# angelini/raft-simulation

Hardware: AMD Instinct MI355X
Metric: simulated node-ticks/sec (5-node Raft) (higher is better)
Workload: dtype u32; 1 GPU; C2: 65,536 5-node clusters/GPU, 10k ticks/step, no faults, no client (steady window); clusters=65536, clusters_per_gpu=65536, nodes=5, parallelism=cluster-sharded x1

## Files before the change

### raft-simulation_amd/csrc/steady_kernel.hip

```cpp
#include <hip/hip_ext.h>

#include "fixed_point_affine.hpp"
#include "tick_wave.hpp"

namespace rs {

constexpr int LANE_WG = 256;

template <int N>
__device__ __forceinline__ uint32_t pick(const uint32_t (&vals)[N], uint32_t k) {
  uint32_t v = 0;
#pragma unroll
  for (int i = 0; i < N; ++i) v |= vals[i] & (0u - (uint32_t)(k == (uint32_t)i));
  return v;
}
__device__ __forceinline__ uint32_t msel(bool a, uint32_t x, uint32_t y) {
  const uint32_t m = 0u - (uint32_t)a;
  return (x & m) | (y & ~m);
}

constexpr int IMG_SLOTS = 32;
constexpr uint32_t IMG_LINE = 64 * 8 * 16;
constexpr uint32_t IMG_HALF = 2 * IMG_LINE;
constexpr uint32_t IMG_WAVE = 2 * IMG_HALF;
// ... 14 lines not shown
}

template <int n>
__host__ __device__ constexpr uint64_t trace_pow() {
  uint64_t x = 1;
  for (int i = 0; i < n; ++i) x *= TRACE_M2;
  return x;
}
template <int n>
__host__ __device__ constexpr uint64_t trace_geo() {
  uint64_t s = 0, x = 1;
  for (int i = 0; i < n; ++i) {
    s += x;
    x *= TRACE_M2;
  }
  return s;
}

static_assert(fpa::M == TRACE_M && fpa::M2 == TRACE_M2 && fpa::ROLE_LEADER == RAFT_LEADER &&
                  fpa::ROLE_FOLLWER == RAFT_FOLLWER &&
                  fpa::EV_APPEND_ENTRIES == RAFT_MSG_APPEND_ENTRIES &&
                  fpa::EV_APPEND_RESPONSE == RAFT_MSG_APPEND_RESPONSE,
              "the affine step's hash is the trace hash");

struct alignas(16) SetWords {
  uint64_t la, lx, ly, lz, fa, fx, fy, fz;
  uint32_t ls, fs, K, K1;
  __device__ __forceinline__ fpa::Half lead() const { return fpa::Half{la, lx, ly, lz, ls}; }
  __device__ __forceinline__ fpa::Half fol() const { return fpa::Half{fa, fx, fy, fz, fs}; }
};
struct BandSets {
  SetWords k[2];
};
__device__ __forceinline__ uint32_t vreg(uint32_t s) {
  uint32_t v;
  asm volatile("v_mov_b32 %0, %1" : "=v"(v) : "s"(s));
  return v;
}
__device__ __forceinline__ uint64_t vreg(uint64_t s) {
  return (uint64_t)vreg((uint32_t)(s >> 32)) << 32 | vreg((uint32_t)s);
}
__device__ __forceinline__ SetWords vreg(const fpa::Set& c, uint32_t K1) {
  return SetWords{vreg(c.lead.a), vreg(c.lead.x), vreg(c.lead.y), vreg(c.lead.z),
                  vreg(c.fol.a),  vreg(c.fol.x),  vreg(c.fol.y),  vreg(c.fol.z),
                  vreg(c.lead.s), vreg(c.fol.s),  vreg(c.K),      vreg(K1)};
}
template <int F>
__device__ __forceinline__ void band_sets(uint32_t nt, uint32_t d, uint32_t hb, BandSets* out) {
  const uint32_t P = fpa::period(F, d, hb), last = 2 * d + F - 1;
  const uint32_t K1 = nt > last ? (nt - last - 1) / P + 1 : 0;
  const fpa::Set lo = fpa::build<F>(d, hb, K1 ? K1 - 1 : 0), hi = fpa::step<F>(lo, d, hb);
  out->k[0] = vreg(lo, K1);
  out->k[1] = vreg(hi, K1);
}

template <int N>
struct FixedPoint {
  static constexpr int F = N - 1;
  uint32_t L, Lid, Lterm, Lcommit;
  uint64_t Ltr, ftr[F];
  uint32_t Ldl, fdl[F], fpend;
  uint32_t qmask, qA[F], qT[F], qa[F], qb[F];
  uint32_t rmask, resA, rT[F], rA[F], rB[F], rH[F];
  uint32_t nhb, nae, nar;

  __device__ __forceinline__ uint32_t fk(int j) const { return (uint32_t)j + ((uint32_t)j >= L ? 1u : 0u); }

  __device__ __forceinline__ void append_entries(uint32_t ta, uint32_t d, uint32_t el_base) {
#pragma unroll
    for (int j = 0; j < F; ++j) {
      ftr[j] = trace_event(ftr[j], ta, RAFT_MSG_APPEND_ENTRIES, Lid, Lterm, RAFT_FOLLWER, Lterm, 0);
      fdl[j] = ta + el_base;
      rT[j] = Lterm; rA[j] = Lcommit; rB[j] = 0; rH[j] = 1;
      qA[j] = INF;
    }
    fpend = (1u << F) - 1;
    qmask = 0;
    rmask = (1u << F) - 1;
    resA = ta + d;
    nae += F;
  }
  __device__ __forceinline__ void responses(uint32_t th, uint32_t tend, uint32_t d, uint32_t hb) {
#pragma unroll
    for (int j = 0; j < F; ++j) {
      const uint32_t tau = th + 2 * d + j;
      if (((rmask >> j) & 1) && tau < tend) {
        Ltr = trace_event(Ltr, tau, RAFT_MSG_APPEND_RESPONSE, fk(j) + 1, Lterm, RAFT_LEADER,
                          Lterm, 0);
        rmask &= ~(1u << j);
        Ldl = tau + hb;
        ++nar;
      }
    }
    if (!rmask) resA = INF;
  }
  __device__ __forceinline__ void rounds(uint32_t th, uint32_t tend, uint32_t d, uint32_t hb,
                                         uint32_t el_base, const BandSets& bs) {
    const uint32_t P = 2 * d + F - 1 + hb, last = 2 * d + F - 1;
    const uint32_t K = tend > th + last ? (tend - th - last - 1) / P + 1 : 0;
    const uint32_t tk = th + K * P;
    if (K) {
      const uint32_t K1 = bs.k[0].K1;
      const bool top = K == K1;
      if (!__builtin_amdgcn_ballot_w64(!top && K + 1 != K1)) {
        const SetWords sw = bs.k[top];
        const fpa::Half cl = sw.lead(), cf = sw.fol();
        Ltr = fpa::apply_leader<F>(cl, Ltr, th, Lterm, L);
        const uint64_t add = fpa::follower_addend<F>(cf, th, Lterm, L);
#pragma unroll
        for (int j = 0; j < F; ++j) ftr[j] = ftr[j] * cf.a + add;
      } else {
        uint64_t a = trace_term(th, 7, 0, 0, RAFT_LEADER, Lterm, 0);
#pragma unroll
        for (int j = 0; j < F; ++j)
          a = a * TRACE_M2 + trace_term(th + 2 * d + j, RAFT_MSG_APPEND_RESPONSE, fk(j) + 1, Lterm,
                                        RAFT_LEADER, Lterm, 0);
        const uint64_t da = (uint64_t)P * (TRACE_M * trace_geo<F + 1>());
        const uint64_t df = (uint64_t)P * TRACE_M;
        uint64_t cf = trace_term(th + d, RAFT_MSG_APPEND_ENTRIES, Lid, Lterm, RAFT_FOLLWER, Lterm, 0);
        for (uint32_t r = 0; r < K; ++r) {
          Ltr = Ltr * trace_pow<F + 1>() + a;
          a += da;
#pragma unroll
          for (int j = 0; j < F; ++j) ftr[j] = ftr[j] * TRACE_M2 + cf;
          cf += df;
        }
      }
#pragma unroll
      for (int j = 0; j < F; ++j) fdl[j] = tk - P + d + el_base;
      fpend = (1u << F) - 1;
      Ldl = tk;
      nhb += K;
      nae += F * K;
      nar += F * K;
    }
    if (tk < tend) {
      Ltr = trace_event(Ltr, tk, 7, 0, 0, RAFT_LEADER, Lterm, 0);
      ++nhb;
      Ldl = tk + hb;
#pragma unroll
      for (int j = 0; j < F; ++j) {
        qA[j] = tk + d; qT[j] = Lterm; qa[j] = Lcommit; qb[j] = 0;
      }
      qmask = (1u << F) - 1;
      if (tk + d < tend) {
        append_entries(tk + d, d, el_base);
        responses(tk, tend, d, hb);
      }
    }
  }
};

template <int N>
__global__ void __launch_bounds__(LANE_WG) steady_lane_kernel(DevSim S, uint32_t t0, uint32_t nt) {
  static_assert(N >= 2 && N <= 5, "follower masks and the response queue fit four followers");
  constexpr int F = N - 1;
  constexpr uint32_t HB = hot_block_words(N);
  constexpr int NWORDS = (int)(HOT_CW + hf_abase(N) * N);
  constexpr int NW4 = (NWORDS + 3) / 4;
  constexpr int IMGC = (int)(HB / 4) < IMG_SLOTS ? (int)(HB / 4) : IMG_SLOTS;
  static_assert(NW4 <= IMGC && IMGC % 8 == 0, "the image holds the words read, in whole lines");
  __shared__ uint32_t bl_c[LANE_WG], bl_t[LANE_WG];
  __shared__ BandSets bs_keep[LANE_WG / 64];
  extern __shared__ __attribute__((aligned(16))) uint32_t dsm[];
  if (blockIdx.x == 0 && threadIdx.x == 0) {
    const uint32_t prev = *S.nbail_zero;
    if (S.bail_report && prev) *S.bail_report = prev;
    if (prev) *S.nbail_zero = 0;
  }
  const uint32_t lane = threadIdx.x & 63, wave = threadIdx.x >> 6;
  const uint32_t cbase = blockIdx.x * LANE_WG + wave * 64;
  const uint32_t c0 = cbase + lane < S.C ? cbase + lane : INF;
  const bool active = c0 != INF;
  const uint32_t c = active ? c0 : 0u;
  const uint32_t g = S.goff + c;
  char* const img = reinterpret_cast<char*>(dsm) + wave * IMG_WAVE;
  uint32_t* const blc = bl_c + wave * 64;
  uint32_t* const blt = bl_t + wave * 64;
  uint32_t nbw = 0;
  auto record_bail = [&](bool b, uint32_t tick) {
    const uint64_t m = __builtin_amdgcn_ballot_w64(b);
    if (b) {
      const uint32_t i = nbw + __builtin_amdgcn_mbcnt_hi((uint32_t)(m >> 32),
                                                         __builtin_amdgcn_mbcnt_lo((uint32_t)m, 0u));
      blc[i] = c;
      blt[i] = tick;
    }
    nbw += (uint32_t)__popcll(m);
  };
#ifdef RS_WAVELOG
  const uint64_t wl_start = wall_clock64();
  uint32_t wl_trips = 0, wl_first = 0, wl_ph[6] = {0, 0, 0, 0, 0, 0};
  uint64_t wl_loop = 0, wl_ts = 0;
#define RS_LPH(i)                                         \
  do {                                                    \
    const uint64_t now_ = __builtin_amdgcn_s_memtime();   \
    wl_ph[i] += (uint32_t)(now_ - wl_ts);                 \
    wl_ts = now_;                                         \
  } while (0)
#else
#define RS_LPH(i) do {} while (0)
#endif

  auto load_wait = [&]() {
    asm volatile("s_waitcnt vmcnt(0)" ::: "memory");
  };
  auto load_line = [&](int ln, bool wait) {
    const uint32_t p = lane & 7;
#pragma unroll
    for (int j = 0; j < 8; ++j) {
      const uint32_t cc = 8 * j + (lane >> 3);
      const uint32_t i = 8 * ln + (p ^ img_sw(cc));
      const uint32_t cg = min(cbase + cc, S.C - 1);
      __builtin_amdgcn_global_load_lds(
          (const __attribute__((address_space(1))) void*)(S.hot + (size_t)cg * HB + 4 * i),
          (__attribute__((address_space(3))) void*)(img + ln * IMG_LINE + j * 1024), 16, 0, 0);
    }
    if (wait) load_wait();
  };
  auto load_half1 = [&]() {
    const uint32_t p = lane & 15;
#pragma unroll
    for (int j = 0; j < 16; ++j) {
      const uint32_t cc = 4 * j + (lane >> 4);
      const uint32_t i = 16 + (p ^ (cc & 15u));
      const uint32_t cg = min(cbase + cc, S.C - 1);
      if (i < (uint32_t)IMGC)
        __builtin_amdgcn_global_load_lds(
            (const __attribute__((address_space(1))) void*)(S.hot + (size_t)cg * HB + 4 * i),
            (__attribute__((address_space(3))) void*)(img + IMG_HALF + j * 1024), 16, 0, 0);
    }
    asm volatile("s_waitcnt vmcnt(0)" ::: "memory");
  };
  static_assert(IMGC >= 16, "lines 0 and 1 are whole in every block");
  uint32_t w[NW4 * 4];
#pragma unroll
  for (int i = 0; i < NW4 * 4; ++i) w[i] = 0;
  load_line(0, false);
  uint32_t nt_s = nt;
  asm volatile("" : "+s"(nt_s));
  const BandSets& bs = bs_keep[wave];
  band_sets<F>(nt_s, S.dmin, S.hb, &bs_keep[wave]);
  load_wait();
#pragma unroll
  for (int i = 0; i < (NW4 < 8 ? NW4 : 8); ++i) {
    const uint4 x = *lds_at<const uint4>(img, img_off(lane, i));
    w[4 * i] = x.x; w[4 * i + 1] = x.y; w[4 * i + 2] = x.z; w[4 * i + 3] = x.w;
  }
  const uint32_t tend = t0 + nt, d = S.dmin;
  const uint32_t P = 2 * d + F - 1 + S.hb, allF = (1u << F) - 1;
  uint32_t dl = 0, nhb = 0, nae = 0, nar = 0;
  bool el = false;
  uint32_t el_to = 0;
#ifdef RS_WAVELOG
  uint64_t wl_x1 = 0, wl_x2 = 0, wl_x3 = 0, wl_lend = 0;
  asm volatile("" ::"v"(w[CL_CERT]), "v"(w[HOT_CW]));
  wl_loop = wall_clock64();
#endif

  static_assert(HOT_CW + (HF_QMETA + 1) * N <= 32 && HF_DEADLINE < HF_QMETA &&
                    HF_TRACE_LO < HF_QMETA && HF_TRACE_HI < HF_QMETA && CL_CTERM < HOT_CW,
                "every word the line-0 path reads is in line 0; REQ_ARR, RES_ARR, the flags and "
                "the term are derived (device.hpp)");
  FixedPoint<N> fx;
  uint32_t lmid = 0, lth0 = 0;
  const bool cfg_ok = S.el_base >= P && S.hb >= 2 * d + F && S.Q >= (uint32_t)F;
  bool strong = active && cfg_ok && (w[CL_CERT] & 0xFFFF0000u) == CERT_STRONG &&
                (w[CL_CERT] & 0xFFFFu) < (uint32_t)N;
  {
    const uint32_t L = w[CL_CERT] & 0xFFFFu;
    auto lw = [&](int f, int k) { return w[HOT_CW + f * N + k]; };
    auto lpick = [&](int f) {
      uint32_t v = 0;
#pragma unroll
      for (int k = 0; k < N; ++k) v |= lw(f, k) & (0u - (uint32_t)(L == (uint32_t)k));
      return v;
    };
    auto lfol = [&](int f, int j) {
      const uint32_t m = 0u - (uint32_t)((uint32_t)j >= L);
      return (lw(f, j + 1) & m) | (lw(f, j) & ~m);
    };
    fx.L = L; fx.Lid = L + 1; fx.Lterm = w[CL_CTERM]; fx.Lcommit = 0;
    fx.Ldl = lpick(HF_DEADLINE);
    fx.Ltr = (uint64_t)lpick(HF_TRACE_HI) << 32 | lpick(HF_TRACE_LO);
    fx.qmask = fx.rmask = 0; fx.resA = INF; fx.fpend = allF; fx.nhb = fx.nae = fx.nar = 0;
    const uint32_t Lqm = lpick(HF_QMETA), rsc = qm_res_cnt(Lqm);
    const uint32_t qm0 = lfol(HF_QMETA, 0);
    const bool need = qm0 != 0;
    strong = strong && (qm0 & ~pack_qmeta(0, 1, 0, 0)) == 0 && Lqm == pack_qmeta(0, 0, 0, rsc) &&
             rsc <= (uint32_t)F && !(need && rsc);
#pragma unroll
    for (int j = 0; j < F; ++j) {
      fx.fdl[j] = lfol(HF_DEADLINE, j);
      fx.ftr[j] = (uint64_t)lfol(HF_TRACE_HI, j) << 32 | lfol(HF_TRACE_LO, j);
      if (j) strong = strong && lfol(HF_QMETA, j) == qm0;
      fx.qA[j] = INF; fx.qT[j] = fx.qa[j] = fx.qb[j] = 0;
      fx.rT[j] = fx.rA[j] = fx.rB[j] = fx.rH[j] = 0;
    }
    lth0 = fx.Ldl;
    if (need) {
      lmid = 1;
      lth0 = fx.Ldl - S.hb;
      const uint32_t ta = lth0 + d;
      strong = strong && fx.Ldl >= S.hb && ta >= t0;
#pragma unroll
      for (int j = 0; j < F; ++j) {
        fx.qA[j] = ta; fx.qT[j] = fx.Lterm;
      }
      fx.qmask = allF;
    } else if (rsc) {
      lmid = 2;
      const uint32_t j0 = (uint32_t)F - rsc, back = S.hb + (j0 ? 2 * d + j0 - 1 : 0u);
      lth0 = fx.Ldl - back;
      const uint32_t ra = lth0 + 2 * d;
      const int64_t cut = (int64_t)t0 - (int64_t)ra;
      strong = strong && fx.Ldl >= back &&
               (int64_t)j0 == (cut < 0 ? 0 : cut > F ? (int64_t)F : cut);
      fx.rmask = allF & ~((1u << j0) - 1);
      fx.resA = ra;
#pragma unroll
      for (int j = 0; j < F; ++j) {
        fx.rT[j] = fx.Lterm; fx.rH[j] = 1;
      }
    } else {
      strong = strong && fx.Ldl >= t0;
    }
    const uint32_t nxt = min((lmid == 2 ? lth0 + P : lth0) + d, tend);
#pragma unroll
    for (int j = 0; j < F; ++j) strong = strong && fx.fdl[j] >= nxt;
  }
  const bool line0_wave = !__builtin_amdgcn_ballot_w64(active && !strong);

  uint32_t Lc = 0;
  bool cert = false, full = false;
  if (!line0_wave) {
    load_line(1, true);
#pragma unroll
    for (int i = 8; i < (NW4 < 16 ? NW4 : 16); ++i) {
      const uint4 x = *lds_at<const uint4>(img, img_off(lane, i));
      w[4 * i] = x.x; w[4 * i + 1] = x.y; w[4 * i + 2] = x.z; w[4 * i + 3] = x.w;
    }
    uint32_t nlc = 0;
#pragma unroll
    for (int k = 0; k < N; ++k) {
      const bool lead = fl_role(w[HOT_CW + HF_FLAGS * N + k]) == RAFT_LEADER;
      Lc = lead ? (uint32_t)k : Lc;
      nlc += lead;
    }
    static_assert(HOT_CW + (HF_FLAGS + 1) * N <= 64, "the flags are in the first two lines");
    cert = active && nlc == 1 &&
           (w[CL_CERT] == (CERT_MAGIC | Lc) || w[CL_CERT] == (CERT_STRONG | Lc));
    full = IMGC > 16 && __builtin_amdgcn_ballot_w64(active && !cert) != 0;
    if (full) {
      load_half1();
#pragma unroll
      for (int i = 16; i < NW4; ++i) {
        const uint4 x = *lds_at<const uint4>(img, img_off(lane, i));
        w[4 * i] = x.x; w[4 * i + 1] = x.y; w[4 * i + 2] = x.z; w[4 * i + 3] = x.w;
      }
    }
  }
  const bool vouched = cert && !full;

  bool lean = strong;
  if (!line0_wave) {
    lean = vouched && cfg_ok;
    lmid = 0;
    const uint32_t L = Lc;
    auto lw = [&](int f, int k) { return w[HOT_CW + f * N + k]; };
    auto lpick = [&](int f) {
      uint32_t v = 0;
#pragma unroll
      for (int k = 0; k < N; ++k) v |= lw(f, k) & (0u - (uint32_t)(L == (uint32_t)k));
      return v;
    };
    auto lfol = [&](int f, int j) {
      const uint32_t m = 0u - (uint32_t)((uint32_t)j >= L);
      return (lw(f, j + 1) & m) | (lw(f, j) & ~m);
    };
    fx.L = L; fx.Lid = L + 1; fx.Lterm = lpick(HF_TERM); fx.Lcommit = 0;
    fx.Ldl = lpick(HF_DEADLINE);
    fx.Ltr = (uint64_t)lpick(HF_TRACE_HI) << 32 | lpick(HF_TRACE_LO);
    fx.qmask = fx.rmask = 0; fx.resA = INF; fx.fpend = allF; fx.nhb = fx.nae = fx.nar = 0;
    const uint32_t Lqm = lpick(HF_QMETA);
    const uint32_t rsc = qm_res_cnt(Lqm);
    uint32_t need = 0;
#pragma unroll
    for (int j = 0; j < F; ++j) {
      fx.fdl[j] = lfol(HF_DEADLINE, j);
      fx.ftr[j] = (uint64_t)lfol(HF_TRACE_HI, j) << 32 | lfol(HF_TRACE_LO, j);
      const uint32_t qm = lfol(HF_QMETA, j);
      lean = lean && (lfol(HF_FLAGS, j) & FL_DRAW) && ((qm >> 4) & 31) <= 1 && !qm_res_cnt(qm);
      need |= (qm_req_cnt(qm) ? 1u : 0u) << j;
      fx.qA[j] = INF; fx.qT[j] = fx.qa[j] = fx.qb[j] = 0;
      fx.rT[j] = fx.rA[j] = fx.rB[j] = fx.rH[j] = 0;
    }
    lean = lean && !qm_req_cnt(Lqm) && rsc <= (uint32_t)F && !(need && rsc) &&
           (need == 0 || need == allF);
    lth0 = fx.Ldl;
    if (need) {
      lmid = 1;
      const uint32_t ta = lfol(HF_REQ_ARR, 0);
      lth0 = ta - d;
      lean = lean && ta >= t0 && ta >= d && fx.Ldl == lth0 + S.hb;
#pragma unroll
      for (int j = 0; j < F; ++j) {
        lean = lean && lfol(HF_REQ_ARR, j) == ta;
        fx.qA[j] = ta; fx.qT[j] = fx.Lterm;
      }
      fx.qmask = allF;
    } else if (rsc) {
      lmid = 2;
      const uint32_t ra = lpick(HF_RES_ARR), j0 = (uint32_t)F - rsc;
      lth0 = ra - 2 * d;
      const int64_t cut = (int64_t)t0 - ((int64_t)lth0 + 2 * d);
      lean = lean && ra >= 2 * d && (int64_t)j0 == (cut < 0 ? 0 : cut > F ? (int64_t)F : cut) &&
             fx.Ldl == (j0 ? lth0 + 2 * d + j0 - 1 : lth0) + S.hb;
      fx.rmask = allF & ~((1u << j0) - 1);
      fx.resA = ra;
#pragma unroll
      for (int j = 0; j < F; ++j) {
        fx.rT[j] = fx.Lterm; fx.rH[j] = 1;
      }
    } else {
      lean = lean && fx.Ldl >= t0;
    }
    const uint32_t nxt = min((lmid == 2 ? lth0 + P : lth0) + d, tend);
#pragma unroll
    for (int j = 0; j < F; ++j) lean = lean && fx.fdl[j] >= nxt;
  }
  const bool lean_wave = !__builtin_amdgcn_ballot_w64(active && !lean);
  bool wb = false;
  if (lean_wave) {
#ifdef RS_WAVELOG
    asm volatile("" ::"v"(fx.Ltr), "v"(fx.fdl[0]), "v"(fx.ftr[0]), "v"(lth0));
    wl_x1 = wl_x2 = wall_clock64();
#endif
    if (active) {
      bool whole = true;
      if (lmid == 1) {
        if (fx.qA[0] < tend) fx.append_entries(fx.qA[0], d, S.el_base);
        else whole = false;
      }
      if (lmid && whole) {
        fx.responses(lth0, tend, d, S.hb);
        whole = !fx.rmask;
      }
      if (whole) fx.rounds(lmid ? lth0 + P : lth0, tend, d, S.hb, S.el_base, bs);
      nhb = fx.nhb; nae = fx.nae; nar = fx.nar;
#ifdef RS_WAVELOG
      asm volatile("" ::"v"(fx.Ltr), "v"(fx.ftr[0]), "v"(fx.Ldl));
      wl_x3 = wall_clock64();
#endif
      const uint32_t L = fx.L;
      uint32_t v[HF_FLAGS][N];
#pragma unroll
      for (int k = 0; k < N; ++k) {
        const bool isL = (uint32_t)k == L;
        const int jl = k > 0 ? k - 1 : 0, jh = k < F ? k : F - 1;
        const bool lo = (uint32_t)k > L;
        auto fv = [&](const uint32_t* x) { return msel(lo, x[jl], x[jh]); };
        const uint32_t fq = (fx.qmask >> (lo ? jl : jh)) & 1, fqa = fv(fx.qA);
        const uint64_t trf = (uint64_t)msel(lo, (uint32_t)(fx.ftr[jl] >> 32),
                                            (uint32_t)(fx.ftr[jh] >> 32)) << 32 |
                             msel(lo, (uint32_t)fx.ftr[jl], (uint32_t)fx.ftr[jh]);
        const uint64_t tr = isL ? fx.Ltr : trf;
        v[HF_DEADLINE][k] = isL ? fx.Ldl : fv(fx.fdl);
        v[HF_TRACE_LO][k] = (uint32_t)tr;
        v[HF_TRACE_HI][k] = (uint32_t)(tr >> 32);
        v[HF_QMETA][k] = isL ? pack_qmeta(0, 0, 0, __popc(fx.rmask)) : pack_qmeta(0, fq, 0, 0);
        v[HF_REQ_ARR][k] = isL ? INF : (fq ? fqa : INF);
        v[HF_RES_ARR][k] = isL ? fx.resA : INF;
        v[HF_REQ_TAIL][k] = isL ? 0u : (fq ? fqa : 0u);
        v[HF_RES_TAIL][k] = isL ? (fx.rmask ? fx.resA : 0u) : 0u;
      }
      static_assert((HOT_CW + HF_FLAGS * N) % 4 == 0 && HOT_CW % 4 == 0, "whole chunks");
      constexpr int CH_END = (int)(HOT_CW + HF_FLAGS * N) / 4;
      auto val = [&](int q) { return v[(q - HOT_CW) / N][(q - HOT_CW) % N]; };
      auto chunk = [&](int i) {
        return make_uint4(val(4 * i), val(4 * i + 1), val(4 * i + 2), val(4 * i + 3));
      };
#pragma unroll
      for (int i = (int)HOT_CW / 4; i < CH_END; ++i) {
        if (i < 8 || !line0_wave) {
          const int q = 4 * i;
          const uint4 x = chunk(i);
          *lds_at<uint4>(img, img_off(lane, i)) = x;
          dl |= (uint32_t)(x.x != w[q] || x.y != w[q + 1] || x.z != w[q + 2] || x.w != w[q + 3])
                << (i / 8);
        }
      }
      if (!line0_wave) {
        const uint32_t cn = CERT_STRONG | L;
        *lds_at<uint4>(img, img_off(lane, CL_CERT / 4)) =
            make_uint4(w[CL_CERT - 3], w[CL_CERT - 2], fx.Lterm, cn);
        static_assert(CL_CTERM == CL_CERT - 1 && CL_CERT % 4 == 3, "one chunk");
        dl |= (uint32_t)(cn != w[CL_CERT] || fx.Lterm != w[CL_CTERM]);
      } else if (CH_END > 8 && (lmid || fx.qmask || fx.rmask)) {
        uint4* const bp = reinterpret_cast<uint4*>(S.hot + (size_t)c * HB);
#pragma unroll
        for (int i = 8; i < CH_END; ++i) bp[i] = chunk(i);
      }
    }
    if (__builtin_amdgcn_ballot_w64(active && (fx.qmask || fx.rmask))) {
#pragma unroll
      for (int j = 0; j < F; ++j) {
        if (active && ((fx.qmask >> j) & 1)) {
          uint4* dp = reinterpret_cast<uint4*>(qslots(S, c * N + fx.fk(j), 0));
          dp[0] = make_uint4(fx.qA[j], RAFT_MSG_APPEND_ENTRIES | fx.Lid << 3, fx.qT[j], fx.qa[j]);
          dp[1] = make_uint4(fx.qb[j], 0, 0, 0);
        }
      }
      uint4* rp = reinterpret_cast<uint4*>(qslots(S, c * N + fx.L, 1));
      uint32_t n = 0;
#pragma unroll
      for (int j = 0; j < F; ++j) {
        if (active && ((fx.rmask >> j) & 1)) {
          uint4* dp = rp + 2 * n;
          dp[0] = make_uint4(fx.resA, RAFT_MSG_APPEND_RESPONSE | (fx.fk(j) + 1) << 3 | fx.rH[j] << 7,
                             fx.rT[j], fx.rA[j]);
          dp[1] = make_uint4(fx.rB[j], 0, 0, 0);
          ++n;
        }
      }
    }
#ifdef RS_WAVELOG
    wl_lend = wall_clock64();
#endif
  } else {
#ifdef RS_WAVELOG
    wl_loop = wall_clock64();
#endif
    auto field = [&](int f, uint32_t (&out)[N]) {
#pragma unroll
      for (int k = 0; k < N; ++k) out[k] = w[HOT_CW + f * N + k];
    };
    {
      auto ifield = [&](int f, int k) { return w[HOT_CW + f * N + k]; };
      bool pat = active && w[CL_HWM_IDX] == 0 && S.Q >= 2u * F && S.el_base >= P && S.hb >= 2 * d + F;
      const uint32_t T = ifield(HF_TERM, 0);
#pragma unroll
      for (int k = 0; k < N; ++k) {
        pat = pat && ifield(HF_FLAGS, k) == 0 && ifield(HF_MASKS, k) == 0 &&
              ifield(HF_TERM, k) == T && ifield(HF_COMMIT, k) == 0 && ifield(HF_LEN, k) == 0 &&
              ifield(HF_QMETA, k) == 0 && ifield(HF_REQ_ARR, k) == INF &&
              ifield(HF_RES_ARR, k) == INF;
#pragma unroll
        for (int p = 0; p < 2 * N; ++p) pat = pat && ifield(HF_NEXT + p, k) == 0;
      }
      pat = pat && T != INF;
      uint32_t cidx = 0, t1 = INF, ntie = 0, bidx = 0;
#pragma unroll
      for (int k = 0; k < N; ++k) {
        const uint32_t dk = ifield(HF_DEADLINE, k);
        cidx = dk < t1 ? (uint32_t)k : cidx;
        t1 = min(t1, dk);
      }
      bool single = true;
#pragma unroll
      for (int k = 0; k < N; ++k) {
        const uint32_t dk = ifield(HF_DEADLINE, k);
        ntie += dk == t1;
        bidx = dk == t1 && (uint32_t)k != cidx ? (uint32_t)k : bidx;
        single = single && ((uint32_t)k == cidx || (uint64_t)dk >= (uint64_t)t1 + d);
      }
      const bool tie = ntie == 2 && d == 1 && N >= 3;
      constexpr uint32_t iL = (N + 1) / 2 >= 2 ? (N + 1) / 2 - 2 : 0;
      const uint64_t tL = (uint64_t)t1 + 2 * d + iL;
      const uint64_t tau0 = max((uint64_t)t1 + 2 * d + F, tL + 2 * d);
      const uint64_t tlast = tau0 + F - 1;
      pat = pat && (single || tie) && t1 >= t0 && (tie || tlast < tend) &&
            (uint64_t)t1 + 4 * N + 8 < 0xFFFFFFFFull;
      if (__builtin_amdgcn_ballot_w64(pat)) {
        const uint32_t* lp = S.hot + (size_t)c * HB + HOT_CW + hf_led(N) * N;
        uint32_t led[N];
#pragma unroll
        for (int k = 0; k < N; ++k) led[k] = lp[k];
#pragma unroll
        for (int k = 0; k < N; ++k) pat = pat && ((uint32_t)k == cidx || led[k] != T + 1);
      }
      const uint32_t T1 = T + 1, cid = cidx + 1, peers = ((1u << (N + 1)) - 1) & ~1u & ~(1u << cid);
      if (pat && single) {
        el = true;
        el_to = 1;
        uint64_t hc = 0;
#pragma unroll
        for (int k = 0; k < N; ++k)
          if ((uint32_t)k == cidx)
            hc = (uint64_t)ifield(HF_TRACE_HI, k) << 32 | ifield(HF_TRACE_LO, k);
        hc = trace_event(hc, t1, 6, 0, 0, RAFT_CANDIDATE, T1, 0);
#pragma unroll
        for (int i = 0; i < F; ++i) {
          const uint32_t sid = (uint32_t)i + ((uint32_t)i >= cidx ? 2u : 1u);
          hc = trace_event(hc, t1 + 2 * d + i, RAFT_MSG_VOTE_RESPONSE, sid, T,
                           (uint32_t)i >= iL ? RAFT_LEADER : RAFT_CANDIDATE, T1, 0);
        }
#pragma unroll
        for (int j = 0; j < F; ++j) {
          const uint32_t sid = (uint32_t)j + ((uint32_t)j >= cidx ? 2u : 1u);
          hc = trace_event(hc, (uint32_t)tau0 + j, RAFT_MSG_APPEND_RESPONSE, sid, T, RAFT_LEADER,
                           T1, 0);
        }
#pragma unroll
        for (int k = 0; k < N; ++k) {
          const bool isc = (uint32_t)k == cidx;
          uint64_t h = (uint64_t)ifield(HF_TRACE_HI, k) << 32 | ifield(HF_TRACE_LO, k);
          h = trace_event(h, t1 + d, RAFT_MSG_REQUEST_VOTE, cid, T1, RAFT_FOLLOWER, T, 0);
          h = trace_event(h, (uint32_t)tL + d, RAFT_MSG_APPEND_ENTRIES, cid, T1, RAFT_FOLLWER, T1, 0);
          h = isc ? hc : h;
          w[HOT_CW + HF_FLAGS * N + k] = isc ? pack_flags(RAFT_LEADER, 0, cid, 0, 0, 1)
                                             : pack_flags(RAFT_FOLLWER, 0, cid, 0, 0, 0) | FL_DRAW;
          w[HOT_CW + HF_MASKS * N + k] = isc ? peers << 16 : 0u;
          w[HOT_CW + HF_TERM * N + k] = T1;
          w[HOT_CW + HF_DEADLINE * N + k] = isc ? (uint32_t)tlast + S.hb
                                                : (uint32_t)tL + d + S.el_base;
          w[HOT_CW + HF_REQ_TAIL * N + k] = 0;
          w[HOT_CW + HF_RES_TAIL * N + k] = 0;
          w[HOT_CW + HF_TRACE_LO * N + k] = (uint32_t)h;
          w[HOT_CW + HF_TRACE_HI * N + k] = (uint32_t)(h >> 32);
        }
        nae = F;
        nar = F;
      } else if (pat && tie) {
        const uint32_t a = cidx, b = bidx, B = b + 1;
        const uint32_t A = cid;
        constexpr uint32_t M = (N + 1) / 2;
        uint64_t ha = 0, hbb = 0;
#pragma unroll
        for (int k = 0; k < N; ++k) {
          const uint64_t h0 = (uint64_t)ifield(HF_TRACE_HI, k) << 32 | ifield(HF_TRACE_LO, k);
          if ((uint32_t)k == a) ha = h0;
          if ((uint32_t)k == b) hbb = h0;
        }
        ha = trace_event(ha, t1, 6, 0, 0, RAFT_CANDIDATE, T1, 0);
        ha = trace_event(ha, t1 + 1, RAFT_MSG_REQUEST_VOTE, B, T1, RAFT_CANDIDATE, T1, 0);
        uint32_t votes = 1, tLt = INF, role = RAFT_CANDIDATE;
#pragma unroll
        for (int k = 0; k < N; ++k) {
          if ((uint32_t)k == a) continue;
          const uint32_t i = (uint32_t)k - ((uint32_t)k > a ? 1u : 0u), tau = t1 + 2 + i;
          const bool grant = (uint32_t)k != b;
          if (grant && role == RAFT_CANDIDATE && ++votes >= M) {
            role = RAFT_LEADER;
            tLt = tau;
          }
          ha = trace_event(ha, tau, RAFT_MSG_VOTE_RESPONSE, (uint32_t)k + 1, grant ? T : T1, role,
                           T1, 0);
        }
        hbb = trace_event(hbb, t1, 6, 0, 0, RAFT_CANDIDATE, T1, 0);
        hbb = trace_event(hbb, t1 + 1, RAFT_MSG_REQUEST_VOTE, A, T1, RAFT_CANDIDATE, T1, 0);
        hbb = trace_event(hbb, t1 + 2, RAFT_MSG_VOTE_RESPONSE, A, T1, RAFT_CANDIDATE, T1, 0);
        uint32_t tb = t1 + 3, j = 0, tbae = INF, brole = RAFT_CANDIDATE, bdl = 0;
        bool bexact = false;
        for (int it = 0; it < N + 1; ++it) {
          const bool res = j < (uint32_t)N - 2, req = tbae == INF;
          if (!res && !req) break;
          if (!res && tb < tLt + 1) tb = tLt + 1;
          const bool rq = req && tb >= tLt + 1;
          bool take_req = rq;
          bexact = false;
          if (res && rq) {
            const uint4 ew = event_draw(g, B, tb, S);
            take_req = !(ew.x & 1);
            bexact = true;
            bdl = tb + S.el_base + __umulhi(ew.y, S.el_span);
          }
          if (take_req) {
            hbb = trace_event(hbb, tb, RAFT_MSG_APPEND_ENTRIES, A, T1, RAFT_FOLLWER, T1, 0);
            brole = RAFT_FOLLWER;
            tbae = tb;
          } else {
            uint32_t fid = 0, cnt = 0;
#pragma unroll
            for (int k = 0; k < N; ++k) {
              const bool other = (uint32_t)k != a && (uint32_t)k != b;
              fid = other && cnt == j ? (uint32_t)k + 1 : fid;
              cnt += other;
            }
            hbb = trace_event(hbb, tb, RAFT_MSG_VOTE_RESPONSE, fid, T, brole, T1, 0);
            ++j;
          }
          if (!bexact) bdl = tb + S.el_base;
// ... 511 lines not shown

#ifdef RS_WAVELOG
    wl_lend = wall_clock64();
#endif
    if (S.shist) {
      const bool kl = wb && run;
      const uint32_t key = kl ? sched_bucket(next_event(), tend) : INF;
      if (kl) S.skey[c] = key;
      uint64_t pend = __builtin_amdgcn_ballot_w64(kl);
      while (pend) {
        const uint32_t k = (uint32_t)__shfl((int)key, (int)__builtin_ctzll(pend));
        const uint64_t same = __builtin_amdgcn_ballot_w64(kl && key == k);
        if (lane == (uint32_t)__builtin_ctzll(pend)) atomicAdd(&S.shist[k], (uint32_t)__popcll(same));
        pend &= ~same;
      }
    }
    const bool wfp = !__builtin_amdgcn_ballot_w64(wb && (!fp || el));
    if (wb) {
      constexpr int NV = HF_NEXT;
      uint32_t v[NV][N];
#pragma unroll
      for (int k = 0; k < N; ++k) {
        const bool isL = (uint32_t)k == L;
        const int jl = k > 0 ? k - 1 : 0, jh = k < F ? k : F - 1;
        const bool lo = (uint32_t)k > L;
        auto fv = [&](const uint32_t* x) { return msel(lo, x[jl], x[jh]); };
        const uint32_t fq = (qmask >> (lo ? jl : jh)) & 1;
        const uint32_t fqa = fv(qA);
        const uint64_t trf = (uint64_t)msel(lo, (uint32_t)(ftr[jl] >> 32), (uint32_t)(ftr[jh] >> 32)) << 32 |
                            msel(lo, (uint32_t)ftr[jl], (uint32_t)ftr[jh]);
        const uint64_t tr = isL ? Ltr : trf;
        v[HF_FLAGS][k] = isL ? Lfl : (fv(ffl) & ~FL_DRAW) | (((fpend >> (lo ? jl : jh)) & 1) ? FL_DRAW : 0u);
        v[HF_MASKS][k] = isL ? Lmk : fv(fmk);
        v[HF_TERM][k] = isL ? Lterm : fv(fterm);
        v[HF_COMMIT][k] = isL ? Lcommit : fv(fcommit);
        v[HF_LEN][k] = isL ? Llen : fv(flen);
        v[HF_DEADLINE][k] = isL ? Ldl : fv(fdl);
        v[HF_QMETA][k] = isL ? pack_qmeta(0, 0, 0, __popc(rmask)) : pack_qmeta(0, fq, 0, 0);
        v[HF_REQ_ARR][k] = isL ? INF : (fq ? fqa : INF);
        v[HF_RES_ARR][k] = isL ? resA : INF;
        v[HF_REQ_TAIL][k] = isL ? 0u : (fq ? fqa : 0u);
        v[HF_RES_TAIL][k] = isL ? (rmask ? resA : 0u) : 0u;
        v[HF_TRACE_LO][k] = (uint32_t)tr;
        v[HF_TRACE_HI][k] = (uint32_t)(tr >> 32);
      }
      auto live = [](int q) { return q >= (int)HOT_CW && q < (int)(HOT_CW + HF_NEXT * N); };
      auto val = [&](int q) { return v[(q - HOT_CW) / N][(q - HOT_CW) % N]; };
      const int ch_end = wfp ? (int)(HOT_CW + (HF_FLAGS + 1) * N + 3) / 4
                             : (int)(HOT_CW + HF_NEXT * N + 3) / 4;
#pragma unroll
      for (int i = (int)HOT_CW / 4; i < (int)(HOT_CW + HF_NEXT * N + 3) / 4; ++i) {
        if (i < ch_end) {
          const int q = 4 * i;
          const uint4 x = make_uint4(live(q) ? val(q) : w[q], live(q + 1) ? val(q + 1) : w[q + 1],
                                     live(q + 2) ? val(q + 2) : w[q + 2],
                                     live(q + 3) ? val(q + 3) : w[q + 3]);
          *lds_at<uint4>(img, img_off(lane, i)) = x;
          dl |= (uint32_t)(x.x != w[q] || x.y != w[q + 1] || x.z != w[q + 2] || x.w != w[q + 3])
                << (i / 8);
        }
      }
      if (el) {
        dl |= (1u << ((HOT_CW + HF_NEXT * N + 31) / 32)) - 1;
        const uint32_t q = HOT_CW + hf_led(N) * N + L;
        if (q < (uint32_t)IMGC * 4) {
          *lds_at<uint32_t>(img, img_off(lane, q / 4) + 4 * (q % 4)) = Lterm;
          dl |= 1u << (q / 32);
        } else {
          S.hot[(size_t)c * HB + q] = Lterm;
        }
      }
      const uint32_t cn = fp || (full && at_fixed_point_state()) ? (CERT_MAGIC | L) : 0u;
      *lds_at<uint4>(img, img_off(lane, CL_CERT / 4)) = make_uint4(w[CL_CERT - 3], w[CL_CERT - 2], w[CL_CERT - 1], cn);
      dl |= (uint32_t)(cn != w[CL_CERT]);
      if (!wfp) {
#pragma unroll
        for (int j = 0; j < F; ++j) {
          const uint32_t qn = HOT_CW + (HF_NEXT + fk(j)) * N + L;
          const uint32_t qt = HOT_CW + (HF_NEXT + N + fk(j)) * N + L;
          if (nx[j] != nx0[j]) {
            *lds_at<uint32_t>(img, img_off(lane, qn / 4) + 4 * (qn % 4)) = (uint32_t)nx[j];
            dl |= 1u << (qn / 32);
          }
          if (mt[j] != mt0[j]) {
            *lds_at<uint32_t>(img, img_off(lane, qt / 4) + 4 * (qt % 4)) = (uint32_t)mt[j];
            dl |= 1u << (qt / 32);
          }
        }
      }
    }
    if (__builtin_amdgcn_ballot_w64(wb && (qmask || rmask))) {
#pragma unroll
      for (int j = 0; j < F; ++j) {
        if (wb && ((qmask >> j) & 1)) {
          uint4* dp = reinterpret_cast<uint4*>(qslots(S, c * N + fk(j), 0));
          dp[0] = make_uint4(qA[j], RAFT_MSG_APPEND_ENTRIES | Lid << 3, qT[j], qa[j]);
          dp[1] = make_uint4(qb[j], 0, 0, 0);
        }
      }
      uint4* rp = reinterpret_cast<uint4*>(qslots(S, c * N + L, 1));
      uint32_t n = 0;
#pragma unroll
      for (int j = 0; j < F; ++j) {
        if (wb && ((rmask >> j) & 1)) {
          const uint32_t sid = fk(j) + 1;
          uint4* dp = rp + 2 * n;
          dp[0] = make_uint4(resA, RAFT_MSG_APPEND_RESPONSE | sid << 3 | rH[j] << 7, rT[j], rA[j]);
          dp[1] = make_uint4(rB[j], 0, 0, 0);
          ++n;
        }
      }
    }
  }
  {
    uint32_t* const wbase = S.hot + (size_t)cbase * HB;
    const uint32_t sub = lane >> 3, q8 = lane & 7;
#pragma unroll
    for (int ln = 0; ln < IMGC / 8; ++ln) {
      const uint64_t bal = __builtin_amdgcn_ballot_w64((dl >> ln) & 1);
      if (!bal) continue;
      uint4 xs[8];
#pragma unroll
      for (int gq = 0; gq < 8; ++gq)
        xs[gq] = *lds_at<const uint4>(img, img_off(8 * gq + sub, 8 * ln + q8));
#pragma unroll
      for (int gq = 0; gq < 8; ++gq) {
        const uint32_t cc = 8 * gq + sub;
        if ((bal >> cc) & 1) {
          typedef uint32_t v4u __attribute__((ext_vector_type(4)));
          const v4u xv = {xs[gq].x, xs[gq].y, xs[gq].z, xs[gq].w};
          uint32_t* const dst = wbase + cc * HB + 4 * (8 * ln + q8);
          asm volatile("global_store_dwordx4 %0, %1, off sc1" : : "v"(dst), "v"(xv) : "memory");
        }
      }
    }
  }
#ifdef RS_WAVELOG
  {
    const uint64_t wl_end = wall_clock64();
    const uint32_t wl_events = nhb + nae + nar;
    const uint32_t emax = ~wave_min(~wl_events), emin = wave_min(wl_events);
    if (lane == 0 && S.wavelog) {
      uint32_t hw, xcc;
      asm volatile("s_getreg_b32 %0, hwreg(HW_REG_HW_ID)" : "=s"(hw));
      asm volatile("s_getreg_b32 %0, hwreg(HW_REG_XCC_ID)" : "=s"(xcc));
      uint4* rec = reinterpret_cast<uint4*>(S.wavelog + (size_t)(blockIdx.x * 4 + wave) * 32);
      rec[0] = make_uint4((uint32_t)wl_start, (uint32_t)(wl_start >> 32), (uint32_t)wl_end,
                          (uint32_t)(wl_end >> 32));
      rec[1] = make_uint4(wl_trips, hw, xcc, wl_first);
      rec[2] = make_uint4((uint32_t)(wl_loop - wl_start), (uint32_t)(wl_lend - wl_start), emin, emax);
      rec[3] = make_uint4(wl_ph[0], wl_ph[1], wl_ph[2], wl_ph[3]);
      rec[4] = make_uint4(wl_ph[4], 0, 0, 0);
      rec[5] = make_uint4((uint32_t)(wl_x1 - wl_start), (uint32_t)(wl_x2 - wl_start),
                          (uint32_t)(wl_x3 - wl_start), 0);
    }
  }
#endif
  {
    const uint32_t h = wave_sum(nhb), a = wave_sum(nae), r = wave_sum(nar);
    unsigned long long* const ctr =
        S.ctr + (size_t)((blockIdx.x * 4 + wave) % CTR_COPIES) * CTR_STRIDE;
    if (lane < 5) {
      const uint32_t msgs = (uint32_t)F * h + a;
      const int idx = lane == 0 ? RAFT_CTR_EV_HEARTBEAT : lane == 1 ? RAFT_CTR_EV_AE
                    : lane == 2 ? RAFT_CTR_EV_AR : lane == 3 ? RAFT_CTR_SENT : RAFT_CTR_DELIVERED;
      const uint32_t v = lane == 0 ? h : lane == 1 ? a : lane == 2 ? r : msgs;
      if (v) atomicAdd(&ctr[idx], (unsigned long long)v);
    }
    if (__builtin_amdgcn_ballot_w64(el)) {
      const uint32_t ne = wave_sum(el ? 1u : 0u), nt = wave_sum(el_to);
      if (lane < 6) {
        const int idx = lane == 0 ? RAFT_CTR_EV_TIMEOUT : lane == 1 ? RAFT_CTR_EV_RV
                      : lane == 2 ? RAFT_CTR_EV_VR : lane == 3 ? RAFT_CTR_LEADERS
                      : lane == 4 ? RAFT_CTR_SENT : RAFT_CTR_DELIVERED;
        const uint32_t v = lane == 0 ? nt : lane == 3 ? ne : lane <= 2 ? (uint32_t)F * nt
                                                                   : (uint32_t)F * (2 * nt + ne);
        atomicAdd(&ctr[idx], (unsigned long long)v);
      }
    }
  }
  if (nbw) {
    if (lane == 0) atomicAdd(S.nbail, nbw);
    asm volatile("s_waitcnt vmcnt(0)" ::: "memory");
    __builtin_amdgcn_fence(__ATOMIC_RELEASE, "workgroup");
    __builtin_amdgcn_fence(__ATOMIC_ACQUIRE, "workgroup");
    tick_wave<N, false, false, true, true>(S, t0, nt, reinterpret_cast<uint32_t*>(img), (int)lane,
                                           0, 1, blc, nbw, blt, blockIdx.x * 4 + wave);
  }
#ifdef RS_WAVELOG
  if (lane == 0 && S.wavelog) {
    const uint64_t wl_done = wall_clock64();
    uint32_t* rec = S.wavelog + (size_t)(blockIdx.x * 4 + wave) * 32;
    rec[17] = (uint32_t)wl_done;
    rec[18] = (uint32_t)(wl_done >> 32);
  }
#endif
}

hipError_t configure_steady() {
  hipError_t e = hipSuccess;
#define RS_CFG(NN)                                                                         \
  if (e == hipSuccess)                                                                     \
    e = hipFuncSetAttribute(reinterpret_cast<const void*>(steady_lane_kernel<NN>),         \
                            hipFuncAttributeMaxDynamicSharedMemorySize,                    \
                            (int)steady_lds_bytes<NN>());
  RS_CFG(2) RS_CFG(3) RS_CFG(4) RS_CFG(5)
#undef RS_CFG
  return e;
}

hipError_t launch_steady(const DevSim& S, uint32_t t0, uint32_t nt, hipStream_t st,
                         hipEvent_t ev0, hipEvent_t ev1) {
  if (S.perm) return hipErrorInvalidValue;
  const dim3 grid((S.C + LANE_WG - 1) / LANE_WG);
  switch (S.N) {
#define RS_LANE(NN)                                                                             \
  case NN:                                                                                      \
    hipExtLaunchKernelGGL((steady_lane_kernel<NN>), grid, dim3(LANE_WG), steady_lds_bytes<NN>(), \
                          st, ev0, ev1, 0, S, t0, nt);                                          \
    break;
    RS_LANE(2) RS_LANE(3) RS_LANE(4) RS_LANE(5)
#undef RS_LANE
    default: return hipErrorInvalidValue;
  }
  return hipGetLastError();
}

}
```

Baseline: 490300 billion node-ticks/s.

## Add node-ordered state for the line-0 fast path, avoiding follower index remapping

Adds a NodeOrder struct for the line-0 steady path that keeps per-node traces indexed by node id rather than by follower slot. This removes the lfol leader-skip selects on load and the per-follower queue arrays, and gives the line-0 path its own write-back and queue emission code. The bail-report bookkeeping now runs after the line-0 load is issued, overlapping it with that load, and the w[] zeroing moves to the slow path. The cost is more duplicated code and register pressure from N traces plus two state structs, and correctness depends on the new per-node update matching the old per-follower one.

After: 525300 billion node-ticks/s (median of 6 runs). 7.1% higher.

```diff
diff --git a/raft-simulation_amd/csrc/steady_kernel.hip b/raft-simulation_amd/csrc/steady_kernel.hip
--- a/raft-simulation_amd/csrc/steady_kernel.hip
+++ b/raft-simulation_amd/csrc/steady_kernel.hip
@@ -190,6 +190,96 @@
 };
 
 template <int N>
+struct NodeOrder {
+  static constexpr int F = N - 1;
+  uint32_t L, T;
+  uint64_t tr[N], Ltr;
+  uint32_t Ldl;
+  bool qin, took;
+  uint32_t qA, fdl;
+  uint32_t rc, resA;
+  uint32_t nhb, nae, nar;
+
+  __device__ __forceinline__ uint32_t sid(int j) const {
+    return (uint32_t)j + 1 + ((uint32_t)j >= L ? 1u : 0u);
+  }
+  __device__ __forceinline__ void followers(uint64_t a, uint64_t add) {
+#pragma unroll
+    for (int k = 0; k < N; ++k) tr[k] = tr[k] * a + add;
+  }
+  __device__ __forceinline__ void append_entries(uint32_t ta, uint32_t d, uint32_t el_base) {
+    followers(TRACE_M2, trace_term(ta, RAFT_MSG_APPEND_ENTRIES, L + 1, T, RAFT_FOLLWER, T, 0));
+    took = true;
+    fdl = ta + el_base;
+    qin = false;
+    rc = F;
+    resA = ta + d;
+    nae += F;
+  }
+  __device__ __forceinline__ void responses(uint32_t th, uint32_t tend, uint32_t d, uint32_t hb) {
+#pragma unroll
+    for (int j = 0; j < F; ++j) {
+      const uint32_t tau = th + 2 * d + j;
+      if ((uint32_t)j + rc >= (uint32_t)F && tau < tend) {
+        Ltr = trace_event(Ltr, tau, RAFT_MSG_APPEND_RESPONSE, sid(j), T, RAFT_LEADER, T, 0);
+        --rc;
+        Ldl = tau + hb;
+        ++nar;
+      }
+    }
+    if (!rc) resA = INF;
+  }
+  __device__ __forceinline__ void rounds(uint32_t th, uint32_t tend, uint32_t d, uint32_t hb,
+                                         uint32_t el_base, const BandSets& bs) {
+    const uint32_t P = 2 * d + F - 1 + hb, last = 2 * d + F - 1;
+    const uint32_t K = tend > th + last ? (tend - th - last - 1) / P + 1 : 0;
+    const uint32_t tk = th + K * P;
+    if (K) {
+      const uint32_t K1 = bs.k[0].K1;
+      const bool top = K == K1;
+      if (!__builtin_amdgcn_ballot_w64(!top && K + 1 != K1)) {
+        const SetWords sw = bs.k[top];
+        const fpa::Half cl = sw.lead(), cf = sw.fol();
+        Ltr = fpa::apply_leader<F>(cl, Ltr, th, T, L);
+        followers(cf.a, fpa::follower_addend<F>(cf, th, T, L));
+      } else {
+        uint64_t a = trace_term(th, 7, 0, 0, RAFT_LEADER, T, 0);
+#pragma unroll
+        for (int j = 0; j < F; ++j)
+          a = a * TRACE_M2 + trace_term(th + 2 * d + j, RAFT_MSG_APPEND_RESPONSE, sid(j), T,
+                                        RAFT_LEADER, T, 0);
+        const uint64_t da = (uint64_t)P * (TRACE_M * trace_geo<F + 1>());
+        const uint64_t df = (uint64_t)P * TRACE_M;
+        uint64_t cf = trace_term(th + d, RAFT_MSG_APPEND_ENTRIES, L + 1, T, RAFT_FOLLWER, T, 0);
+        for (uint32_t r = 0; r < K; ++r) {
+          Ltr = Ltr * trace_pow<F + 1>() + a;
+          a += da;
+          followers(TRACE_M2, cf);
+          cf += df;
+        }
+      }
+      took = true;
+      fdl = tk - P + d + el_base;
+      Ldl = tk;
+      nhb += K;
+      nae += F * K;
+      nar += F * K;
+    }
+    if (tk < tend) {
+      Ltr = trace_event(Ltr, tk, 7, 0, 0, RAFT_LEADER, T, 0);
+      ++nhb;
+      Ldl = tk + hb;
+      qin = true;
+      qA = tk + d;
+      if (tk + d < tend) {
+        append_entries(tk + d, d, el_base);
+        responses(tk, tend, d, hb);
+      }
+    }
+  }
+};
+
+template <int N>
 __global__ void __launch_bounds__(LANE_WG) steady_lane_kernel(DevSim S, uint32_t t0, uint32_t nt) {
   static_assert(N >= 2 && N <= 5, "follower masks and the response queue fit four followers");
   constexpr int F = N - 1;
@@ -201,11 +291,6 @@
   __shared__ uint32_t bl_c[LANE_WG], bl_t[LANE_WG];
   __shared__ BandSets bs_keep[LANE_WG / 64];
   extern __shared__ __attribute__((aligned(16))) uint32_t dsm[];
-  if (blockIdx.x == 0 && threadIdx.x == 0) {
-    const uint32_t prev = *S.nbail_zero;
-    if (S.bail_report && prev) *S.bail_report = prev;
-    if (prev) *S.nbail_zero = 0;
-  }
   const uint32_t lane = threadIdx.x & 63, wave = threadIdx.x >> 6;
   const uint32_t cbase = blockIdx.x * LANE_WG + wave * 64;
   const uint32_t c0 = cbase + lane < S.C ? cbase + lane : INF;
@@ -272,16 +357,23 @@
   };
   static_assert(IMGC >= 16, "lines 0 and 1 are whole in every block");
   uint32_t w[NW4 * 4];
-#pragma unroll
-  for (int i = 0; i < NW4 * 4; ++i) w[i] = 0;
+  asm volatile("" ::"s"(nt), "s"(t0), "s"(S.dmin), "s"(S.hb), "s"(S.el_base));
   load_line(0, false);
+  const bool reporter = blockIdx.x == 0 && threadIdx.x == 0;
+  uint32_t prev_bails = 0;
+  if (reporter) prev_bails = *S.nbail_zero;
   uint32_t nt_s = nt;
   asm volatile("" : "+s"(nt_s));
   const BandSets& bs = bs_keep[wave];
   band_sets<F>(nt_s, S.dmin, S.hb, &bs_keep[wave]);
   load_wait();
-#pragma unroll
-  for (int i = 0; i < (NW4 < 8 ? NW4 : 8); ++i) {
+  if (reporter && prev_bails) {
+    if (S.bail_report) *S.bail_report = prev_bails;
+    *S.nbail_zero = 0;
+  }
+  static_assert(NW4 >= 8, "line 0 is read whole");
+#pragma unroll
+  for (int i = 0; i < 8; ++i) {
     const uint4 x = *lds_at<const uint4>(img, img_off(lane, i));
     w[4 * i] = x.x; w[4 * i + 1] = x.y; w[4 * i + 2] = x.z; w[4 * i + 3] = x.w;
   }
@@ -292,6 +384,7 @@
   uint32_t el_to = 0;
 #ifdef RS_WAVELOG
   uint64_t wl_x1 = 0, wl_x2 = 0, wl_x3 = 0, wl_lend = 0;
+  uint32_t wl_cut = 0;
   asm volatile("" ::"v"(w[CL_CERT]), "v"(w[HOT_CW]));
   wl_loop = wall_clock64();
 #endif
@@ -300,7 +393,7 @@
                     HF_TRACE_LO < HF_QMETA && HF_TRACE_HI < HF_QMETA && CL_CTERM < HOT_CW,
                 "every word the line-0 path reads is in line 0; REQ_ARR, RES_ARR, the flags and "
                 "the term are derived (device.hpp)");
-  FixedPoint<N> fx;
+  NodeOrder<N> no;
   uint32_t lmid = 0, lth0 = 0;
   const bool cfg_ok = S.el_base >= P && S.hb >= 2 * d + F && S.Q >= (uint32_t)F;
   bool strong = active && cfg_ok && (w[CL_CERT] & 0xFFFF0000u) == CERT_STRONG &&
@@ -314,65 +407,139 @@
       for (int k = 0; k < N; ++k) v |= lw(f, k) & (0u - (uint32_t)(L == (uint32_t)k));
       return v;
     };
-    auto lfol = [&](int f, int j) {
-      const uint32_t m = 0u - (uint32_t)((uint32_t)j >= L);
-      return (lw(f, j + 1) & m) | (lw(f, j) & ~m);
-    };
-    fx.L = L; fx.Lid = L + 1; fx.Lterm = w[CL_CTERM]; fx.Lcommit = 0;
-    fx.Ldl = lpick(HF_DEADLINE);
-    fx.Ltr = (uint64_t)lpick(HF_TRACE_HI) << 32 | lpick(HF_TRACE_LO);
-    fx.qmask = fx.rmask = 0; fx.resA = INF; fx.fpend = allF; fx.nhb = fx.nae = fx.nar = 0;
+    no.L = L; no.T = w[CL_CTERM];
+    no.Ldl = lpick(HF_DEADLINE);
+    no.Ltr = (uint64_t)lpick(HF_TRACE_HI) << 32 | lpick(HF_TRACE_LO);
+#pragma unroll
+    for (int k = 0; k < N; ++k) no.tr[k] = (uint64_t)lw(HF_TRACE_HI, k) << 32 | lw(HF_TRACE_LO, k);
+    no.qin = no.took = false; no.qA = no.fdl = 0; no.rc = 0; no.resA = INF;
+    no.nhb = no.nae = no.nar = 0;
     const uint32_t Lqm = lpick(HF_QMETA), rsc = qm_res_cnt(Lqm);
-    const uint32_t qm0 = lfol(HF_QMETA, 0);
+    const uint32_t qm0 = L ? lw(HF_QMETA, 0) : lw(HF_QMETA, 1);
     const bool need = qm0 != 0;
     strong = strong && (qm0 & ~pack_qmeta(0, 1, 0, 0)) == 0 && Lqm == pack_qmeta(0, 0, 0, rsc) &&
              rsc <= (uint32_t)F && !(need && rsc);
 #pragma unroll
-    for (int j = 0; j < F; ++j) {
-      fx.fdl[j] = lfol(HF_DEADLINE, j);
-      fx.ftr[j] = (uint64_t)lfol(HF_TRACE_HI, j) << 32 | lfol(HF_TRACE_LO, j);
-      if (j) strong = strong && lfol(HF_QMETA, j) == qm0;
-      fx.qA[j] = INF; fx.qT[j] = fx.qa[j] = fx.qb[j] = 0;
-      fx.rT[j] = fx.rA[j] = fx.rB[j] = fx.rH[j] = 0;
-    }
-    lth0 = fx.Ldl;
+    for (int k = 0; k < N; ++k) strong = strong && (L == (uint32_t)k || lw(HF_QMETA, k) == qm0);
+    lth0 = no.Ldl;
     if (need) {
       lmid = 1;
-      lth0 = fx.Ldl - S.hb;
+      lth0 = no.Ldl - S.hb;
       const uint32_t ta = lth0 + d;
-      strong = strong && fx.Ldl >= S.hb && ta >= t0;
-#pragma unroll
-      for (int j = 0; j < F; ++j) {
-        fx.qA[j] = ta; fx.qT[j] = fx.Lterm;
-      }
-      fx.qmask = allF;
+      strong = strong && no.Ldl >= S.hb && ta >= t0;
+      no.qin = true;
+      no.qA = ta;
     } else if (rsc) {
       lmid = 2;
       const uint32_t j0 = (uint32_t)F - rsc, back = S.hb + (j0 ? 2 * d + j0 - 1 : 0u);
-      lth0 = fx.Ldl - back;
+      lth0 = no.Ldl - back;
       const uint32_t ra = lth0 + 2 * d;
       const int64_t cut = (int64_t)t0 - (int64_t)ra;
-      strong = strong && fx.Ldl >= back &&
+      strong = strong && no.Ldl >= back &&
                (int64_t)j0 == (cut < 0 ? 0 : cut > F ? (int64_t)F : cut);
-      fx.rmask = allF & ~((1u << j0) - 1);
-      fx.resA = ra;
+      no.rc = rsc;
+      no.resA = ra;
+    } else {
+      strong = strong && no.Ldl >= t0;
+    }
+    const uint32_t nxt = min((lmid == 2 ? lth0 + P : lth0) + d, tend);
+#pragma unroll
+    for (int k = 0; k < N; ++k)
+      strong = strong && (L == (uint32_t)k || lw(HF_DEADLINE, k) >= nxt);
+  }
+  const bool line0_wave = !__builtin_amdgcn_ballot_w64(active && !strong);
+  if (line0_wave) {
+#ifdef RS_WAVELOG
+    asm volatile("" ::"v"(no.Ltr), "v"(no.Ldl), "v"(no.tr[0]), "v"(lth0));
+    wl_x1 = wl_x2 = wall_clock64();
+#endif
+    if (active) {
+      bool whole = true;
+      if (lmid == 1) {
+        if (no.qA < tend) no.append_entries(no.qA, d, S.el_base);
+        else whole = false;
+      }
+      if (lmid && whole) {
+        no.responses(lth0, tend, d, S.hb);
+        whole = !no.rc;
+      }
+      if (whole) no.rounds(lmid ? lth0 + P : lth0, tend, d, S.hb, S.el_base, bs);
+      nhb = no.nhb; nae = no.nae; nar = no.nar;
+#ifdef RS_WAVELOG
+      asm volatile("" ::"v"(no.Ltr), "v"(no.tr[0]), "v"(no.Ldl));
+      wl_x3 = wall_clock64();
+#endif
+      const uint32_t fqm = pack_qmeta(0, no.qin ? 1u : 0u, 0, 0), Lqm = pack_qmeta(0, 0, 0, no.rc);
+      const uint32_t fra = no.qin ? no.qA : INF, frt = no.qin ? no.qA : 0u;
+      const uint32_t Lrt = no.rc ? no.resA : 0u;
+      auto val = [&](int q) -> uint32_t {
+        const int f = (q - (int)HOT_CW) / N, k = (q - (int)HOT_CW) % N;
+        const bool isL = no.L == (uint32_t)k;
+        switch (f) {
+          case HF_DEADLINE: return isL ? no.Ldl : no.took ? no.fdl : w[q];
+          case HF_TRACE_LO: return (uint32_t)(isL ? no.Ltr : no.tr[k]);
+          case HF_TRACE_HI: return (uint32_t)((isL ? no.Ltr : no.tr[k]) >> 32);
+          case HF_QMETA: return isL ? Lqm : fqm;
+          case HF_REQ_ARR: return isL ? INF : fra;
+          case HF_RES_ARR: return isL ? no.resA : INF;
+          case HF_REQ_TAIL: return isL ? 0u : frt;
+          default: return isL ? Lrt : 0u;
+        }
+      };
+      static_assert(HF_RES_TAIL + 1 == HF_FLAGS, "the fields written: DEADLINE .. RES_TAIL");
+      static_assert((HOT_CW + HF_FLAGS * N) % 4 == 0 && HOT_CW % 4 == 0, "whole chunks");
+      constexpr int CH_END = (int)(HOT_CW + HF_FLAGS * N) / 4;
+      auto chunk = [&](int i) {
+        return make_uint4(val(4 * i), val(4 * i + 1), val(4 * i + 2), val(4 * i + 3));
+      };
+#pragma unroll
+      for (int i = (int)HOT_CW / 4; i < (CH_END < 8 ? CH_END : 8); ++i) {
+        const int q = 4 * i;
+        const uint4 x = chunk(i);
+        *lds_at<uint4>(img, img_off(lane, i)) = x;
+        dl |= (uint32_t)(x.x != w[q] || x.y != w[q + 1] || x.z != w[q + 2] || x.w != w[q + 3]);
+      }
+      if (CH_END > 8 && (lmid || no.qin || no.rc)) {
+        uint4* const bp = reinterpret_cast<uint4*>(S.hot + (size_t)c * HB);
+#pragma unroll
+        for (int i = 8; i < CH_END; ++i) bp[i] = chunk(i);
+      }
+    }
+    if (__builtin_amdgcn_ballot_w64(active && (no.qin || no.rc))) {
+      if (active && no.qin) {
+#pragma unroll
+        for (int k = 0; k < N; ++k) {
+          if (no.L != (uint32_t)k) {
+            uint4* dp = reinterpret_cast<uint4*>(qslots(S, c * N + k, 0));
+            dp[0] = make_uint4(no.qA, RAFT_MSG_APPEND_ENTRIES | (no.L + 1) << 3, no.T, 0);
+            dp[1] = make_uint4(0, 0, 0, 0);
+          }
+        }
+      }
+      uint4* rp = reinterpret_cast<uint4*>(qslots(S, c * N + no.L, 1));
+      uint32_t n = 0;
 #pragma unroll
       for (int j = 0; j < F; ++j) {
-        fx.rT[j] = fx.Lterm; fx.rH[j] = 1;
-      }
-    } else {
-      strong = strong && fx.Ldl >= t0;
-    }
-    const uint32_t nxt = min((lmid == 2 ? lth0 + P : lth0) + d, tend);
-#pragma unroll
-    for (int j = 0; j < F; ++j) strong = strong && fx.fdl[j] >= nxt;
-  }
-  const bool line0_wave = !__builtin_amdgcn_ballot_w64(active && !strong);
+        if (active && (uint32_t)j + no.rc >= (uint32_t)F) {
+          uint4* dp = rp + 2 * n;
+          dp[0] = make_uint4(no.resA, RAFT_MSG_APPEND_RESPONSE | no.sid(j) << 3 | 1u << 7, no.T, 0);
+          dp[1] = make_uint4(0, 0, 0, 0);
+          ++n;
+        }
+      }
+    }
+#ifdef RS_WAVELOG
+    wl_lend = wall_clock64();
+    wl_cut = __builtin_amdgcn_ballot_w64(active && (lmid || no.qin || no.rc)) ? 1u : 0u;
+#endif
+  }
 
   uint32_t Lc = 0;
   bool cert = false, full = false;
   if (!line0_wave) {
     load_line(1, true);
+#pragma unroll
+    for (int i = 32; i < NW4 * 4; ++i) w[i] = 0;
 #pragma unroll
     for (int i = 8; i < (NW4 < 16 ? NW4 : 16); ++i) {
       const uint4 x = *lds_at<const uint4>(img, img_off(lane, i));
@@ -400,7 +567,8 @@
   }
   const bool vouched = cert && !full;
 
-  bool lean = strong;
+  FixedPoint<N> fx;
+  bool lean = false;
   if (!line0_wave) {
     lean = vouched && cfg_ok;
     lmid = 0;
@@ -467,7 +635,7 @@
 #pragma unroll
     for (int j = 0; j < F; ++j) lean = lean && fx.fdl[j] >= nxt;
   }
-  const bool lean_wave = !__builtin_amdgcn_ballot_w64(active && !lean);
+  const bool lean_wave = !line0_wave && !__builtin_amdgcn_ballot_w64(active && !lean);
   bool wb = false;
   if (lean_wave) {
 #ifdef RS_WAVELOG
@@ -520,25 +688,17 @@
       };
 #pragma unroll
       for (int i = (int)HOT_CW / 4; i < CH_END; ++i) {
-        if (i < 8 || !line0_wave) {
-          const int q = 4 * i;
-          const uint4 x = chunk(i);
-          *lds_at<uint4>(img, img_off(lane, i)) = x;
-          dl |= (uint32_t)(x.x != w[q] || x.y != w[q + 1] || x.z != w[q + 2] || x.w != w[q + 3])
-                << (i / 8);
-        }
-      }
-      if (!line0_wave) {
-        const uint32_t cn = CERT_STRONG | L;
-        *lds_at<uint4>(img, img_off(lane, CL_CERT / 4)) =
-            make_uint4(w[CL_CERT - 3], w[CL_CERT - 2], fx.Lterm, cn);
-        static_assert(CL_CTERM == CL_CERT - 1 && CL_CERT % 4 == 3, "one chunk");
-        dl |= (uint32_t)(cn != w[CL_CERT] || fx.Lterm != w[CL_CTERM]);
-      } else if (CH_END > 8 && (lmid || fx.qmask || fx.rmask)) {
-        uint4* const bp = reinterpret_cast<uint4*>(S.hot + (size_t)c * HB);
-#pragma unroll
-        for (int i = 8; i < CH_END; ++i) bp[i] = chunk(i);
-      }
+        const int q = 4 * i;
+        const uint4 x = chunk(i);
+        *lds_at<uint4>(img, img_off(lane, i)) = x;
+        dl |= (uint32_t)(x.x != w[q] || x.y != w[q + 1] || x.z != w[q + 2] || x.w != w[q + 3])
+              << (i / 8);
+      }
+      const uint32_t cn = CERT_STRONG | L;
+      *lds_at<uint4>(img, img_off(lane, CL_CERT / 4)) =
+          make_uint4(w[CL_CERT - 3], w[CL_CERT - 2], fx.Lterm, cn);
+      static_assert(CL_CTERM == CL_CERT - 1 && CL_CERT % 4 == 3, "one chunk");
+      dl |= (uint32_t)(cn != w[CL_CERT] || fx.Lterm != w[CL_CTERM]);
     }
     if (__builtin_amdgcn_ballot_w64(active && (fx.qmask || fx.rmask))) {
 #pragma unroll
@@ -565,7 +725,7 @@
 #ifdef RS_WAVELOG
     wl_lend = wall_clock64();
 #endif
-  } else {
+  } else if (!line0_wave) {
 #ifdef RS_WAVELOG
     wl_loop = wall_clock64();
 #endif
@@ -1383,7 +1543,7 @@
       rec[3] = make_uint4(wl_ph[0], wl_ph[1], wl_ph[2], wl_ph[3]);
       rec[4] = make_uint4(wl_ph[4], 0, 0, 0);
       rec[5] = make_uint4((uint32_t)(wl_x1 - wl_start), (uint32_t)(wl_x2 - wl_start),
-                          (uint32_t)(wl_x3 - wl_start), 0);
+                          (uint32_t)(wl_x3 - wl_start), wl_cut);
     }
   }
 #endif
```
